# SamsungLabs/nb-asr

Hardware: AMD Instinct MI355X
Metric: utterances_per_sec (higher is better)
Workload: dtype f32

## Files before the change

### nb_asr_amd/csrc/gemm_pointwise.hip

```cpp
#include "storage.h"

namespace nbasr {

typedef float floatx4 __attribute__((ext_vector_type(4)));
typedef _Float16 pw_h2 __attribute__((ext_vector_type(2)));

constexpr int PW_M = 128, PW_N = 256, PW_K = 32;
constexpr int PW_THREADS = 512;

__device__ __forceinline__ float pw_load(const float* p) { return *p; }
__device__ __forceinline__ float pw_load(const bf16_t* p) { return __uint_as_float(static_cast<unsigned>(p->bits) << 16); }
__device__ __forceinline__ void pw_store(float* p, float v) { *p = v; }
__device__ __forceinline__ void pw_store(bf16_t* p, float v) { p->bits = static_cast<unsigned short>(pack_bf16x2(v, 0.f) & 0xffffu); }

template <int TERMS>
struct PwSteps {
    static constexpr int NS = TERMS;
    static constexpr int A_STEP = TERMS * 2 * 2 * PW_M * 16;
    static constexpr int X_STEP = TERMS * 2 * 2 * PW_N * 16;
    static constexpr int RING = 3;
    static constexpr int LDS = RING * (A_STEP + X_STEP);
    static constexpr int DMA_PER_WAVE = 3 * TERMS;
};

// ... 82 lines not shown


template <bool LNX, class T>
__device__ __forceinline__ void pw_fetch32(const T* __restrict__ x, int c_in, int frames, int ld, const LnRef& ln, float (&v)[PW_K])
{
    const int ci0 = blockIdx.y * PW_K, b = blockIdx.z;
    const int t = blockIdx.x * PW_N + threadIdx.x;
    const bool live = t < frames;
    const T* __restrict__ xb = x + static_cast<size_t>(b) * c_in * ld + t;
    float mean = 0.f, rstd = 0.f;
    if (LNX && live) {
        const float* st = ln.stats + static_cast<size_t>(b) * 2 * ld;
        mean = st[t]; rstd = st[ld + t];
    }
#pragma unroll
    for (int c = 0; c < PW_K; ++c) {
        const int ci = ci0 + c;
        v[c] = (live && ci < c_in) ? pw_load(xb + static_cast<size_t>(ci) * ld) : 0.f;
    }
    if (LNX) {
#pragma unroll
        for (int c = 0; c < PW_K; ++c) {
            const int ci = ci0 + c;
            if (live && ci < c_in) v[c] = ln_apply(v[c], mean, rstd, ln.gamma[ci], ln.beta[ci]);
        }
    }
}

template <bool LNX>
__global__ __launch_bounds__(256) void pw_tile_max_kernel(const float* __restrict__ x, float* __restrict__ partial, int c_in,
                                                          int frames, int ld, int n_ks, const LnRef ln)
{
    __shared__ float s_max[4];
    float v[PW_K];
    pw_fetch32<LNX>(x, c_in, frames, ld, ln, v);
    float m = 0.f;
#pragma unroll
    for (int c = 0; c < PW_K; ++c) m = fmaxf(m, fabsf(v[c]));
#pragma unroll
    for (int d = 32; d >= 1; d >>= 1) m = fmaxf(m, __shfl_xor(m, d));
    if ((threadIdx.x & 63) == 0) s_max[threadIdx.x >> 6] = m;
    __syncthreads();
    if (threadIdx.x == 0)
        partial[(static_cast<size_t>(blockIdx.z) * gridDim.x + blockIdx.x) * n_ks + blockIdx.y] = fmaxf(fmaxf(s_max[0], s_max[1]), fmaxf(s_max[2], s_max[3]));
}

template <class P, bool LNX>
__global__ __launch_bounds__(256) void pw_presplit_kernel(const typename P::act_t* __restrict__ x, unsigned char* __restrict__ image,
                                                          float* __restrict__ inv_scale, const float* __restrict__ partial,
                                                          int c_in, int frames, int ld, int n_ks, const LnRef ln)
{
    const int nt = blockIdx.x, ks = blockIdx.y, b = blockIdx.z;
    const int lane_t = threadIdx.x;
    float v[PW_K];
    pw_fetch32<LNX>(x, c_in, frames, ld, ln, v);
    float scale = 1.f;
    if constexpr (P::SCALED) {
        const float* __restrict__ pt = partial + (static_cast<size_t>(b) * gridDim.x + nt) * n_ks;
        float tile_max = 0.f;
        for (int i = threadIdx.x & 63; i < n_ks; i += 64) tile_max = fmaxf(tile_max, pt[i]);
#pragma unroll
        for (int d = 32; d >= 1; d >>= 1) tile_max = fmaxf(tile_max, __shfl_xor(tile_max, d));
        float inv;
        pw_pow2(tile_max, 14, scale, inv);
        if (threadIdx.x == 0 && ks == 0) inv_scale[static_cast<size_t>(b) * gridDim.x + nt] = inv;
    }
    unsigned char* step = image + ((static_cast<size_t>(b) * gridDim.x + nt) * n_ks + ks) * P::X_STEP;
#pragma unroll
    for (int bh = 0; bh < 4; ++bh) {
        u4v term[P::NS];
#pragma unroll
// ... 425 lines not shown
```

### nb_asr_amd/csrc/layernorm.hip

```cpp
#include "storage.h"

namespace nbasr {

constexpr int LN_ROWS = 16;
constexpr int LN_QS = 16;

template <typename T, bool MINMAX = false, int FR = Chunk<T>::FR>
__device__ __forceinline__ void tile_statistics(const T* x, int channels, int ld, float eps, size_t base, bool active,
                                                int row, int ql, float (*s_mean)[LN_QS * FR], float (*s_m2)[LN_QS * FR],
                                                float* s_cnt, float* s_mu, float* s_rstd,
                                                float (*s_lo)[LN_QS * FR] = nullptr, float (*s_hi)[LN_QS * FR] = nullptr)
{
    float shift[FR], s1[FR], s2[FR], lo[FR], hi[FR];
#pragma unroll
    for (int r = 0; r < FR; ++r) { shift[r] = 0.f; s1[r] = 0.f; s2[r] = 0.f; lo[r] = 3.0e38f; hi[r] = -3.0e38f; }
    int n = 0;
    if (active && row < channels) {
        load_frames<FR>(x + base + static_cast<size_t>(row) * ld, shift);
        auto fold = [&](const float (&e)[FR]) {
#pragma unroll
            for (int r = 0; r < FR; ++r) {
                const float d = e[r] - shift[r];
                s1[r] += d;
                s2[r] = __builtin_fmaf(d, d, s2[r]);
                if (MINMAX) { lo[r] = fminf(lo[r], e[r]); hi[r] = fmaxf(hi[r], e[r]); }
            }
            ++n;
        };
        int c = row;
        for (; c + 7 * LN_ROWS < channels; c += 8 * LN_ROWS) {
            float e[8][FR];
#pragma unroll
            for (int u = 0; u < 8; ++u) load_frames<FR>(x + base + static_cast<size_t>(c + u * LN_ROWS) * ld, e[u]);
#pragma unroll
            for (int u = 0; u < 8; ++u) fold(e[u]);
        }
        for (; c + 3 * LN_ROWS < channels; c += 4 * LN_ROWS) {
            float e[4][FR];
#pragma unroll
            for (int u = 0; u < 4; ++u) load_frames<FR>(x + base + static_cast<size_t>(c + u * LN_ROWS) * ld, e[u]);
#pragma unroll
            for (int u = 0; u < 4; ++u) fold(e[u]);
        }
        for (; c < channels; c += LN_ROWS) {
            float e[FR];
            load_frames<FR>(x + base + static_cast<size_t>(c) * ld, e);
            fold(e);
        }
    }
    const float fn = static_cast<float>(n);
#pragma unroll
    for (int r = 0; r < FR; ++r) {
        const float dm = n ? s1[r] / fn : 0.f;
        s_mean[row][ql * FR + r] = shift[r] + dm;
        s_m2[row][ql * FR + r] = n ? fmaxf(s2[r] - dm * s1[r], 0.f) : 0.f;
        if (MINMAX) { s_lo[row][ql * FR + r] = lo[r]; s_hi[row][ql * FR + r] = hi[r]; }
    }
    if (ql == 0) s_cnt[row] = fn;
    __syncthreads();

    if (threadIdx.x < LN_QS * FR) {
        const int col = threadIdx.x;
        float cnt = 0.f, mean = 0.f, m2 = 0.f;
#pragma unroll
        for (int k = 0; k < LN_ROWS; ++k) {
            const float nb = s_cnt[k];
            if (nb > 0.f) {
                const float tot = cnt + nb;
                const float delta = s_mean[k][col] - mean;
                mean += delta * (nb / tot);
                m2 += s_m2[k][col] + delta * delta * (cnt * nb / tot);
                cnt = tot;
            }
        }
        s_mu[col] = mean;
        s_rstd[col] = 1.0f / sqrtf(m2 / fmaxf(cnt, 1.f) + eps);
        if (MINMAX) {
            float l = s_lo[0][col], h = s_hi[0][col];
#pragma unroll
            for (int k = 1; k < LN_ROWS; ++k) { l = fminf(l, s_lo[k][col]); h = fmaxf(h, s_hi[k][col]); }
            s_lo[0][col] = l; s_hi[0][col] = h;
        }
    }
    __syncthreads();
}

template <typename TI, typename TO, bool ABSMAX>
__global__ __launch_bounds__(256) void layernorm_channels_kernel(
    const TI* x, const float* __restrict__ gamma, const float* __restrict__ beta,
    TO* y, int channels, int frames, int ld, float eps, unsigned* __restrict__ absmax)
{
    constexpr int FR = Chunk<TI>::FR;
    __shared__ float s_mean[LN_ROWS][LN_QS * FR];
    __shared__ float s_m2[LN_ROWS][LN_QS * FR];
// ... 88 lines not shown
    NBASR_REQUIRE(x && gamma && beta && y, NBASR_ENULL, "%s: NULL pointer", what);
    NBASR_REQUIRE(aligned16(x) && aligned16(y), NBASR_EALIGN, "%s: x, y must be 16-byte aligned", what);
    NBASR_REQUIRE(batch <= 65535, NBASR_EINVAL, "%s: batch %d > 65535", what, batch);
    NBASR_REQUIRE(!absmax || in_dtype == NBASR_F32, NBASR_EINVAL, "%s: the absmax by-product exists for fp32 tensors only", what);
    const int nq = ld / fr;
    const dim3 grid((nq + LN_QS - 1) / LN_QS, batch);
    if (in_dtype == NBASR_BF16) {
        if (out_dtype == NBASR_BF16)
            hipLaunchKernelGGL((layernorm_channels_kernel<bf16_t, bf16_t, false>), grid, dim3(256), 0, as_stream(stream),
                               static_cast<const bf16_t*>(x), gamma, beta, static_cast<bf16_t*>(y), channels, frames, ld, eps, static_cast<unsigned*>(nullptr));
        else
            hipLaunchKernelGGL((layernorm_channels_kernel<bf16_t, float, false>), grid, dim3(256), 0, as_stream(stream),
                               static_cast<const bf16_t*>(x), gamma, beta, static_cast<float*>(y), channels, frames, ld, eps, static_cast<unsigned*>(nullptr));
    } else if (absmax) {
        zero_async(absmax, sizeof(float) * batch, as_stream(stream));
        hipLaunchKernelGGL((layernorm_channels_kernel<float, float, true>), grid, dim3(256), 0, as_stream(stream),
                           static_cast<const float*>(x), gamma, beta, static_cast<float*>(y), channels, frames, ld, eps, reinterpret_cast<unsigned*>(absmax));
    } else {
        hipLaunchKernelGGL((layernorm_channels_kernel<float, float, false>), grid, dim3(256), 0, as_stream(stream),
                           static_cast<const float*>(x), gamma, beta, static_cast<float*>(y), channels, frames, ld, eps, static_cast<unsigned*>(nullptr));
    }
    return launch_status(what);
}

extern "C" int nbasr_layernorm_channels(const void* x, const float* gamma, const float* beta, void* y, float* absmax, int batch,
                                        int channels, int frames, int ld, float eps, int in_dtype, int out_dtype, nbasr_stream_t stream)
{
    clear_error();
    NBASR_REQUIRE(!absmax || (in_dtype == NBASR_F32 && out_dtype == NBASR_F32), NBASR_EINVAL,
                  "nbasr_layernorm_channels: the max|y| by-product exists for fp32 -> fp32 only");
    return layernorm_impl("nbasr_layernorm_channels", x, gamma, beta, y, absmax, batch, channels, frames, ld, eps, stream, in_dtype, out_dtype);
}

__global__ __launch_bounds__(256) void channel_stats_bound_kernel(const float* __restrict__ x, const float* __restrict__ gamma,
                                                                  const float* __restrict__ beta, float* __restrict__ stats,
                                                                  unsigned* __restrict__ bound, int channels, int frames, int ld, float eps)
{
    __shared__ float s_mean[LN_ROWS][LN_QS * 4];
    __shared__ float s_m2[LN_ROWS][LN_QS * 4];
    __shared__ float s_cnt[LN_ROWS];
    __shared__ float s_mu[LN_QS * 4];
    __shared__ float s_rstd[LN_QS * 4];
    __shared__ float s_gb[8];
    __shared__ float s_lo[LN_ROWS][LN_QS * 4];
    __shared__ float s_hi[LN_ROWS][LN_QS * 4];

    const int ql = threadIdx.x & (LN_QS - 1);
    const int row = threadIdx.x / LN_QS;
    const int nq = ld >> 2;
    const int q = blockIdx.x * LN_QS + ql;
    const int b = blockIdx.y;
    const bool active = q < nq;
    const size_t base = static_cast<size_t>(b) * channels * ld + static_cast<size_t>(q) * 4;

    float gm = 0.f, bm = 0.f;
    for (int c = threadIdx.x; c < channels; c += 256) { gm = fmaxf(gm, fabsf(gamma[c])); bm = fmaxf(bm, fabsf(beta[c])); }
#pragma unroll
    for (int d = 32; d >= 1; d >>= 1) { gm = fmaxf(gm, __shfl_xor(gm, d)); bm = fmaxf(bm, __shfl_xor(bm, d)); }
    if ((threadIdx.x & 63) == 0) { s_gb[threadIdx.x >> 6] = gm; s_gb[4 + (threadIdx.x >> 6)] = bm; }

    tile_statistics<float, true>(x, channels, ld, eps, base, active, row, ql, s_mean, s_m2, s_cnt, s_mu, s_rstd, s_lo, s_hi);
    gm = fmaxf(fmaxf(s_gb[0], s_gb[1]), fmaxf(s_gb[2], s_gb[3]));
    bm = fmaxf(fmaxf(s_gb[4], s_gb[5]), fmaxf(s_gb[6], s_gb[7]));

    float dev = 0.f;
    if (threadIdx.x < LN_QS * 4) {
        const int t = blockIdx.x * (LN_QS * 4) + threadIdx.x;
        if (t < ld) {
            const bool live = t < frames;
            float* srow = stats + static_cast<size_t>(b) * 2 * ld;
            srow[t] = live ? s_mu[threadIdx.x] : 0.f;
            srow[ld + t] = live ? s_rstd[threadIdx.x] : 0.f;
            if (live) dev = finite_abs(fmaxf(s_hi[0][threadIdx.x] - s_mu[threadIdx.x], s_mu[threadIdx.x] - s_lo[0][threadIdx.x]) * s_rstd[threadIdx.x]);
        }
    }
    if (threadIdx.x < 64) {
#pragma unroll
        for (int d = 32; d >= 1; d >>= 1) dev = fmaxf(dev, __shfl_xor(dev, d));
        if (threadIdx.x == 0) atomicMax(bound + b, __float_as_uint(finite_abs((dev * gm + bm) * 1.0001f)));
    }
}

template <bool NORM>
__global__ __launch_bounds__(256) void normalize_split_kernel(const float* __restrict__ x, const float* __restrict__ stats,
                                                              const float* __restrict__ gamma, const float* __restrict__ beta,
                                                              const float* __restrict__ bound, unsigned char* __restrict__ image,
                                                              int channels, int , int ld,
                                                              int bound_stride)
{
    typedef _Float16 halfx8 __attribute__((ext_vector_type(8)));
    constexpr int SPLIT_PITCH = 68;
    __shared__ __attribute__((aligned(16))) unsigned char s_tile[4][2][4 * SPLIT_PITCH * 16];
    const int ql = threadIdx.x & 63, wv = threadIdx.x >> 6, oct0 = wv + 4 * blockIdx.z;
    const int nq = ld >> 2;
    const int q = blockIdx.x * 64 + ql;
    const int b = blockIdx.y;
    const int n_groups = (channels + 15) >> 4;
    const size_t rows = static_cast<size_t>(ld) + 1;
    unsigned char* const img_b = image + static_cast<size_t>(b) * n_groups * 4 * rows * 16;
    if (blockIdx.x == 0 && blockIdx.z == 0) {
        const uint4 z = make_uint4(0u, 0u, 0u, 0u);
        for (int pl = threadIdx.x; pl < n_groups * 4; pl += 256) *reinterpret_cast<uint4*>(img_b + static_cast<size_t>(pl) * rows * 16) = z;
    }
    if (blockIdx.x * 64 >= nq) return;
    const bool inside = q < nq;
    float scale = 1.f;
    {
        const unsigned bits = __float_as_uint(bound[static_cast<size_t>(b) * bound_stride]);
        const int e = static_cast<int>((bits >> 23) & 0xffu);
        int k = (bits & 0x7fffffffu) ? (127 + 14) - e : 0;
        k = k > 126 ? 126 : (k < -126 ? -126 : k);
        scale = __uint_as_float(static_cast<unsigned>(127 + k) << 23);
// ... 67 lines not shown
            const int f = 64 * k + ql;
            if (blockIdx.x * 256 + f < ld) {
                *reinterpret_cast<halfx8*>(plane_hi + f * 16) = hi;
                *reinterpret_cast<halfx8*>(plane_lo + f * 16) = lo;
            }
        }
        asm volatile("s_waitcnt lgkmcnt(0)" ::: "memory");
#pragma unroll
        for (int c = 0; c < 8; ++c) cur[c] = nxt[c];
    }
}

static int split_grid_z(int tiles, int batch)
{
    const long long wgs = static_cast<long long>(tiles) * batch;
    int z = 4;
    while (z < 16 && wgs * z < 512) z *= 2;
    return z;
}

extern "C" int nbasr_layernorm_split_image(const float* x, const float* gamma, const float* beta, float* stats, float* bound,
                                           void* image, int batch, int channels, int frames, int ld, float eps,
                                           nbasr_stream_t stream)
{
    clear_error();
    NBASR_REQUIRE(batch >= 0 && channels > 0 && frames >= 0, NBASR_EINVAL, "nbasr_layernorm_split_image: bad sizes");
    NBASR_REQUIRE(ld >= frames && ld % 4 == 0, NBASR_EALIGN, "nbasr_layernorm_split_image: ld=%d must be >= frames=%d and a multiple of 4", ld, frames);
    if (batch == 0 || ld == 0) return NBASR_OK;
    NBASR_REQUIRE(x && gamma && beta && stats && bound && image, NBASR_ENULL, "nbasr_layernorm_split_image: NULL pointer");
    NBASR_REQUIRE(aligned16(x) && aligned16(stats) && aligned16(image), NBASR_EALIGN, "nbasr_layernorm_split_image: x, stats, image must be 16-byte aligned");
    NBASR_REQUIRE(batch <= 65535, NBASR_EINVAL, "nbasr_layernorm_split_image: batch %d > 65535", batch);
    zero_async(bound, sizeof(float) * batch, as_stream(stream));
    const int nq = ld / 4;
    hipLaunchKernelGGL(channel_stats_bound_kernel, dim3((nq + LN_QS - 1) / LN_QS, batch), dim3(256), 0, as_stream(stream),
                       x, gamma, beta, stats, reinterpret_cast<unsigned*>(bound), channels, frames, ld, eps);
    hipLaunchKernelGGL(normalize_split_kernel<true>, dim3((nq + 63) / 64, batch, split_grid_z((nq + 63) / 64, batch)), dim3(256), 0, as_stream(stream),
                       x, stats, gamma, beta, bound, static_cast<unsigned char*>(image), channels, frames, ld, 1);
    return launch_status("nbasr_layernorm_split_image");
}

__global__ __launch_bounds__(256) void input_range_kernel(const float* __restrict__ x, unsigned* __restrict__ range,
                                                          int channels, int frames, int ld)
{
    __shared__ float s_max[4][256];
    __shared__ unsigned s_bad[4];
    const int b = blockIdx.y;
    const int lane = threadIdx.x & 63, slice = threadIdx.x >> 6;
    const int t0 = (blockIdx.x * 64 + lane) * 4;
    float m[4] = {0.f, 0.f, 0.f, 0.f};
    unsigned bad = 0u;
    if (t0 < frames) {
        const float* col = x + static_cast<size_t>(b) * channels * ld + t0;
        const bool whole = t0 + 4 <= ld && ld % 4 == 0 && (reinterpret_cast<size_t>(x) & 15) == 0;
        for (int c = slice; c < channels; c += 4) {
            float v[4] = {0.f, 0.f, 0.f, 0.f};
            if (whole) {
                const float4 q = *reinterpret_cast<const float4*>(col + static_cast<size_t>(c) * ld);
                v[0] = q.x; v[1] = q.y; v[2] = q.z; v[3] = q.w;
            } else {
#pragma unroll
                for (int r = 0; r < 4; ++r) if (t0 + r < frames) v[r] = col[static_cast<size_t>(c) * ld + r];
            }
#pragma unroll
            for (int r = 0; r < 4; ++r) {
                const float a = fabsf(v[r]);
                if (t0 + r < frames) {
                    if (!(a <= 3.4028234664e38f)) bad = 1u;
                    else m[r] = fmaxf(m[r], a);
                }
            }
        }
    }
#pragma unroll
    for (int r = 0; r < 4; ++r) s_max[slice][lane * 4 + r] = m[r];
#pragma unroll
    for (int d = 32; d >= 1; d >>= 1) bad |= __shfl_xor(bad, d);
    if (lane == 0) s_bad[slice] = bad;
    __syncthreads();
    const int t = blockIdx.x * 256 + threadIdx.x;
    const float fmax_ = fmaxf(fmaxf(s_max[0][threadIdx.x], s_max[1][threadIdx.x]), fmaxf(s_max[2][threadIdx.x], s_max[3][threadIdx.x]));
    float hi = fmax_, lo = (t < frames && fmax_ > 0.f) ? fmax_ : __uint_as_float(0x7f800000u);
#pragma unroll
    for (int d = 32; d >= 1; d >>= 1) {
        hi = fmaxf(hi, __shfl_xor(hi, d));
        lo = fminf(lo, __shfl_xor(lo, d));
    }
    if (lane == 0) {
        atomicMax(range + 4 * b, __float_as_uint(hi));
        atomicMin(range + 4 * b + 1, __float_as_uint(lo));
        if (slice == 0 && (s_bad[0] | s_bad[1] | s_bad[2] | s_bad[3])) atomicOr(range + 4 * b + 2, 0x3f800000u);
    }
}

__global__ void input_range_init_kernel(unsigned* __restrict__ range, int batch)
{
    const int b = blockIdx.x * blockDim.x + threadIdx.x;
    if (b < batch) { range[4 * b] = 0u; range[4 * b + 1] = 0x7f800000u; range[4 * b + 2] = 0u; range[4 * b + 3] = 0u; }
}

extern "C" int nbasr_input_range(const float* x, float* range, int batch, int channels, int frames, int ld, nbasr_stream_t stream)
{
    clear_error();
    NBASR_REQUIRE(batch >= 0 && channels > 0 && frames >= 0 && ld >= frames, NBASR_EINVAL, "nbasr_input_range: bad sizes");
    if (batch == 0) return NBASR_OK;
    NBASR_REQUIRE(range, NBASR_ENULL, "nbasr_input_range: range is NULL");
    NBASR_REQUIRE(batch <= 65535, NBASR_EINVAL, "nbasr_input_range: batch %d > 65535", batch);
    hipLaunchKernelGGL(input_range_init_kernel, dim3((batch + 255) / 256), dim3(256), 0, as_stream(stream), reinterpret_cast<unsigned*>(range), batch);
    if (frames > 0) {
        NBASR_REQUIRE(x, NBASR_ENULL, "nbasr_input_range: x is NULL");
        hipLaunchKernelGGL(input_range_kernel, dim3((frames + 255) / 256, batch), dim3(256), 0, as_stream(stream), x,
                           reinterpret_cast<unsigned*>(range), channels, frames, ld);
    }
    return launch_status("nbasr_input_range");
}

extern "C" int nbasr_split_image_ranged(const float* x, const float* x_range, void* image, int batch, int channels, int frames,
                                        int ld, nbasr_stream_t stream)
{
    clear_error();
    NBASR_REQUIRE(batch >= 0 && channels > 0 && frames >= 0, NBASR_EINVAL, "nbasr_split_image_ranged: bad sizes");
    NBASR_REQUIRE(ld >= frames && ld % 4 == 0, NBASR_EALIGN, "nbasr_split_image_ranged: ld=%d must be >= frames=%d and a multiple of 4", ld, frames);
    if (batch == 0 || ld == 0) return NBASR_OK;
    NBASR_REQUIRE(x && x_range && image, NBASR_ENULL, "nbasr_split_image_ranged: NULL pointer");
    NBASR_REQUIRE(aligned16(x) && aligned16(image), NBASR_EALIGN, "nbasr_split_image_ranged: x, image must be 16-byte aligned");
    NBASR_REQUIRE(batch <= 65535, NBASR_EINVAL, "nbasr_split_image_ranged: batch %d > 65535", batch);
    const int nq = ld / 4;
    hipLaunchKernelGGL(normalize_split_kernel<false>, dim3((nq + 63) / 64, batch, split_grid_z((nq + 63) / 64, batch)), dim3(256), 0, as_stream(stream),
                       x, static_cast<const float*>(nullptr), static_cast<const float*>(nullptr), static_cast<const float*>(nullptr),
                       x_range, static_cast<unsigned char*>(image), channels, frames, ld, 4);
    return launch_status("nbasr_split_image_ranged");
}

extern "C" int nbasr_channel_stats(const void* x, float* stats, int batch, int channels, int frames, int ld, float eps, int dtype,
                                     nbasr_stream_t stream)
{
    clear_error();
    NBASR_REQUIRE(dtype == NBASR_F32 || dtype == NBASR_BF16, NBASR_EINVAL, "nbasr_channel_stats: unknown dtype %d", dtype);
    NBASR_REQUIRE(batch >= 0 && channels > 0 && frames >= 0, NBASR_EINVAL, "nbasr_channel_stats: bad sizes");
    const int fr = dtype == NBASR_BF16 ? 8 : 4;
    NBASR_REQUIRE(ld >= frames && ld % fr == 0, NBASR_EALIGN, "nbasr_channel_stats: ld=%d must be >= frames=%d and a multiple of %d", ld, frames, fr);
    if (batch == 0 || ld == 0) return NBASR_OK;
    NBASR_REQUIRE(x && stats, NBASR_ENULL, "nbasr_channel_stats: NULL pointer");
    NBASR_REQUIRE(aligned16(x) && aligned16(stats), NBASR_EALIGN, "nbasr_channel_stats: x, stats must be 16-byte aligned");
// ... 129 lines not shown
```

### nb_asr_amd/csrc/lstm.hip

```cpp
#include "common.h"

#include <cstdlib>
#include <mutex>
#include <vector>

namespace nbasr {

constexpr int NBASR_MAX_DEVICES = 64;

typedef float floatx4 __attribute__((ext_vector_type(4)));

int lstm_input_projection(const float* x, const float* w_ih, const float* b_ih, const float* b_hh, float* gates,
                          int batch, int c_in, int frames, int ld, int rows4h, LnRef ln, hipStream_t stream);

__device__ __forceinline__ float sigmoidf_(float v) { return 1.0f / (1.0f + expf(-v)); }

constexpr int LSTM_WAVES = 8;
constexpr int LSTM_CHUNKS = 4;

constexpr int LSTMP_HU = 8;

__global__ __launch_bounds__(256) void lstm_pack_whh_kernel(const float* __restrict__ w_hh, float4* __restrict__ packed, int hidden,
                                                            int slices, int kchunks_p)
{
// ... 54 lines not shown
            for (int c = 0; c < LSTM_CHUNKS; ++c) {
#pragma unroll
                for (int m = 0; m < 2; ++m) acc[m] = __builtin_amdgcn_mfma_f32_16x16x4f32(wv[c][m].x, hv[c].x, acc[m], 0, 0, 0);
#pragma unroll
                for (int m = 0; m < 2; ++m) acc[m] = __builtin_amdgcn_mfma_f32_16x16x4f32(wv[c][m].y, hv[c].y, acc[m], 0, 0, 0);
#pragma unroll
                for (int m = 0; m < 2; ++m) acc[m] = __builtin_amdgcn_mfma_f32_16x16x4f32(wv[c][m].z, hv[c].z, acc[m], 0, 0, 0);
#pragma unroll
                for (int m = 0; m < 2; ++m) acc[m] = __builtin_amdgcn_mfma_f32_16x16x4f32(wv[c][m].w, hv[c].w, acc[m], 0, 0, 0);
            }
        }
    }
#pragma unroll
    for (int m = 0; m < 2; ++m)
#pragma unroll
        for (int r = 0; r < 4; ++r) red[wave][m][r][lane] = acc[m][r];
    __syncthreads();

    if (!e_ok) return;
    const int mt = jj >> 2, pl = (jj & 3) * 16 + bb;
#pragma unroll
    for (int g = 0; g < 4; ++g) {
        float s = red[0][mt][g][pl];
#pragma unroll
        for (int w = 1; w < LSTM_WAVES; ++w) s += red[w][mt][g][pl];
        pre[g] += s;
    }
    const float c_new = sigmoidf_(pre[1]) * c_prev + sigmoidf_(pre[0]) * tanhf(pre[2]);
    const float h_new = sigmoidf_(pre[3]) * tanhf(c_new);
    cell[static_cast<size_t>(eb) * hidden + ej] = c_new;
    h_out[(static_cast<size_t>(eb) * frames + t) * hidden + ej] = h_new;
}

template <bool BCT>
__global__ __launch_bounds__(256) void head_kernel(
    const float* __restrict__ h, const float* __restrict__ w, const float* __restrict__ bias,
    float* __restrict__ out, int rows, int features, int classes, int frames, int ld, const LnRef ln)
{
    const int lane = threadIdx.x & 63, wave = threadIdx.x >> 6;
    const int i16 = lane & 15, kq = lane >> 4;
    const int r0 = (blockIdx.x * 4 + wave) * 16;
    if (r0 >= rows) return;

    floatx4 acc[4], part[4];
#pragma unroll
    for (int n = 0; n < 4; ++n) { acc[n] = floatx4{0.f, 0.f, 0.f, 0.f}; part[n] = floatx4{0.f, 0.f, 0.f, 0.f}; }

    const int row = r0 + i16;
    const bool row_ok = row < rows;
    const int kchunks = (features + 15) / 16;
    for (int c = 0; c < kchunks; ++c) {
        if ((c & 7) == 0 && c) {
#pragma unroll
            for (int n = 0; n < 4; ++n) { acc[n] += part[n]; part[n] = floatx4{0.f, 0.f, 0.f, 0.f}; }
        }
        const int k = c * 16 + kq * 4;
        const bool kok = k < features;
        float av[4] = {0.f, 0.f, 0.f, 0.f};
        if (row_ok && kok) {
            if (!BCT) {
                const float4 v = *reinterpret_cast<const float4*>(h + static_cast<size_t>(row) * features + k);
                av[0] = v.x; av[1] = v.y; av[2] = v.z; av[3] = v.w;
            } else {
                const int bb = row / frames, tt = row - bb * frames;
                const float* p = h + (static_cast<size_t>(bb) * features + k) * ld + tt;
#pragma unroll
                for (int e = 0; e < 4; ++e) av[e] = p[static_cast<size_t>(e) * ld];
                if (ln.stats) {
                    const float* st = ln.stats + static_cast<size_t>(bb) * 2 * ld;
                    const float mean = st[tt], rstd = st[ld + tt];
#pragma unroll
                    for (int e = 0; e < 4; ++e) av[e] = ln_apply(av[e], mean, rstd, ln.gamma[k + e], ln.beta[k + e]);
                }
            }
        }
#pragma unroll
        for (int n = 0; n < 4; ++n) {
            const int cls = n * 16 + i16;
            float4 wv = make_float4(0.f, 0.f, 0.f, 0.f);
            if (cls < classes && kok) wv = *reinterpret_cast<const float4*>(w + static_cast<size_t>(cls) * features + k);
            part[n] = __builtin_amdgcn_mfma_f32_16x16x4f32(av[0], wv.x, part[n], 0, 0, 0);
            part[n] = __builtin_amdgcn_mfma_f32_16x16x4f32(av[1], wv.y, part[n], 0, 0, 0);
            part[n] = __builtin_amdgcn_mfma_f32_16x16x4f32(av[2], wv.z, part[n], 0, 0, 0);
            part[n] = __builtin_amdgcn_mfma_f32_16x16x4f32(av[3], wv.w, part[n], 0, 0, 0);
        }
    }
#pragma unroll
    for (int n = 0; n < 4; ++n) acc[n] += part[n];
#pragma unroll
    for (int n = 0; n < 4; ++n) {
        const int cls = n * 16 + i16;
        if (cls >= classes) continue;
        const float bv = bias[cls];
#pragma unroll
        for (int r = 0; r < 4; ++r) {
            const int rr = r0 + kq * 4 + r;
            if (rr < rows) out[static_cast<size_t>(rr) * classes + cls] = acc[n][r] + bv;
        }
    }
}

constexpr int LSTMS_QUADS = LSTM_WAVES * LSTM_CHUNKS * 4;
constexpr int LSTMS_IMAGE_FLOATS = LSTMS_QUADS * 16 * 4;
constexpr int LSTMS_HEADER_WORDS = 64;
constexpr unsigned long long LSTMS_TIMEOUT_TICKS = 100000000ull;

typedef unsigned lstm_u4 __attribute__((ext_vector_type(4)));

__device__ __forceinline__ unsigned lstm_tag(int t) { return (static_cast<unsigned>((t >> 1) + 1) & 1u) << 30; }

__global__ __launch_bounds__(64 * LSTM_WAVES) void lstm_seq_kernel(
    const float* __restrict__ gates_in,
    const float4* __restrict__ wp,
    float* __restrict__ cell, float* __restrict__ h_out, unsigned* status, float* hx,
    int batch, int frames, int hidden, int kchunks_p, int flags)
{
    __shared__ float4 red[2][LSTM_WAVES][2][64];
    __shared__ int stop;
    if ((flags & NBASR_LSTM_SEQ_INJECT_FAULT) && blockIdx.x == 0) return;

    const int lane = threadIdx.x & 63, wave = __builtin_amdgcn_readfirstlane(threadIdx.x >> 6);
    const int i16 = lane & 15, kq = lane >> 4;
    const int slice = blockIdx.x, tile = blockIdx.y;
    const int b0 = tile * 16;
    if (threadIdx.x == 0) stop = 0;

    float4 wv[LSTM_CHUNKS][2];
    {
        const bool mine = wave * LSTM_CHUNKS < kchunks_p;
        const float4* wslice = wp + (static_cast<size_t>(slice) * kchunks_p + (mine ? wave * LSTM_CHUNKS : 0)) * 2 * 64 + lane;
#pragma unroll
// ... 269 lines not shown
    } else {
        hipLaunchKernelGGL(lstm_seq_kernel, grid, block, 0, as_stream(stream), gates_ws, static_cast<const float4*>(packed_whh), cell_ws, h_out,
                           words, hx, batch, frames, hidden, lstm_kchunks_p(hidden), flags);
    }
    e = hipEventRecord(done, as_stream(stream));
    if (e != hipSuccess) { set_error("nbasr_lstm_recurrence_seq: hipEventRecord: %s", hipGetErrorString(e)); return static_cast<int>(e); }
    return launch_status("nbasr_lstm_recurrence_seq");
}

extern "C" int nbasr_lstm_seq_status(const void* seq_ws, nbasr_stream_t stream)
{
    clear_error();
    NBASR_REQUIRE(seq_ws, NBASR_ENULL, "nbasr_lstm_seq_status: NULL pointer");
    unsigned word = 0;
    hipError_t e = hipMemcpyAsync(&word, seq_ws, sizeof(word), hipMemcpyDeviceToHost, as_stream(stream));
    if (e == hipSuccess) e = hipStreamSynchronize(as_stream(stream));
    if (e != hipSuccess) { set_error("nbasr_lstm_seq_status: %s", hipGetErrorString(e)); return static_cast<int>(e); }
    NBASR_REQUIRE(word == 0, NBASR_EINVAL, "nbasr_lstm_seq_status: a step of the one-launch recurrence timed out waiting for its peers "
                  "(status %u): the grid was not co-resident", word);
    return NBASR_OK;
}

extern "C" int nbasr_linear_head(const float* h, const float* w, const float* bias, float* logits, int rows,
                                 int features, int classes, nbasr_stream_t stream)
{
    clear_error();
    NBASR_REQUIRE(rows >= 0 && features > 0 && classes > 0 && classes <= 64, NBASR_EINVAL,
                  "nbasr_linear_head: rows=%d features=%d classes=%d (classes must be <= 64)", rows, features, classes);
    if (rows == 0) return NBASR_OK;
    NBASR_REQUIRE(h && w && bias && logits, NBASR_ENULL, "nbasr_linear_head: NULL pointer");
    NBASR_REQUIRE(features % 4 == 0 && aligned16(h) && aligned16(w), NBASR_EALIGN,
                  "nbasr_linear_head: features must be a multiple of 4 and h, w 16-byte aligned");
    if (rows == 0) return NBASR_OK;
    hipLaunchKernelGGL(head_kernel<false>, dim3((rows + 63) / 64), dim3(256), 0, as_stream(stream),
                       h, w, bias, logits, rows, features, classes, 0, 0, LnRef{nullptr, nullptr, nullptr});
    return launch_status("nbasr_linear_head");
}

extern "C" int nbasr_linear_head_bct(const float* x, const float* w, const float* bias, float* logits, int batch,
                                     int features, int frames, int ld, int classes, const nbasr_deferred_ln* ln,
                                     nbasr_stream_t stream)
{
    clear_error();
    NBASR_REQUIRE(batch >= 0 && features > 0 && frames >= 0 && ld >= frames && classes > 0 && classes <= 64, NBASR_EINVAL,
                  "nbasr_linear_head_bct: bad sizes (classes must be <= 64)");
    if (batch == 0 || frames == 0) return NBASR_OK;
    NBASR_REQUIRE(x && w && bias && logits, NBASR_ENULL, "nbasr_linear_head_bct: NULL pointer");
    NBASR_REQUIRE(features % 4 == 0 && aligned16(w), NBASR_EALIGN, "nbasr_linear_head_bct: features must be a multiple of 4, w 16-byte aligned");
    NBASR_REQUIRE(!ln || (ln->stats && ln->gamma && ln->beta), NBASR_ENULL, "nbasr_linear_head_bct: deferred LayerNorm needs stats, gamma and beta");
    const long long rows = static_cast<long long>(batch) * frames;
    if (rows == 0) return NBASR_OK;
    hipLaunchKernelGGL(head_kernel<true>, dim3(static_cast<unsigned>((rows + 63) / 64)), dim3(256), 0, as_stream(stream),
                       x, w, bias, logits, static_cast<int>(rows), features, classes, frames, ld, ln_ref(ln, true));
    return launch_status("nbasr_linear_head_bct");
}
```

Measured before the change: 11470.

## Vectorize tile-max fetch, widen stats/range kernels with XCD tiling, LDS-stage head GEMM

The pointwise tile-max kernel gains a float4 fast path for aligned inputs. The channel-stats and input-range kernels move to wider 512/256-thread blocks with XCD-contiguous tile remapping, and the range kernel gets a deeper load unroll. The linear head kernel is rewritten to stage weight and activation tiles in LDS, with register prefetch of the next K block, so weights are reused across waves. Together these aim to cut memory traffic and latency in several small kernels, at the cost of more LDS, extra synchronisation and more code complexity.

```diff
diff --git a/nb_asr_amd/csrc/gemm_pointwise.hip b/nb_asr_amd/csrc/gemm_pointwise.hip
--- a/nb_asr_amd/csrc/gemm_pointwise.hip
+++ b/nb_asr_amd/csrc/gemm_pointwise.hip
@@ -138,11 +138,45 @@
                                                           int frames, int ld, int n_ks, const LnRef ln)
 {
     __shared__ float s_max[4];
-    float v[PW_K];
-    pw_fetch32<LNX>(x, c_in, frames, ld, ln, v);
     float m = 0.f;
-#pragma unroll
-    for (int c = 0; c < PW_K; ++c) m = fmaxf(m, fabsf(v[c]));
+    if (ld % 4 == 0 && ((reinterpret_cast<size_t>(x) | (LNX ? reinterpret_cast<size_t>(ln.stats) : 0)) & 15) == 0) {
+        const int ci0 = blockIdx.y * PW_K + (threadIdx.x >> 6) * (PW_K / 4), b = blockIdx.z;
+        const int t0 = blockIdx.x * PW_N + (threadIdx.x & 63) * 4;
+        if (t0 < frames) {
+            const float* __restrict__ xb = x + static_cast<size_t>(b) * c_in * ld + t0;
+            float4 q[PW_K / 4];
+#pragma unroll
+            for (int c = 0; c < PW_K / 4; ++c) {
+                const int ci = ci0 + c;
+                q[c] = ci < c_in ? *reinterpret_cast<const float4*>(xb + static_cast<size_t>(ci) * ld) : make_float4(0.f, 0.f, 0.f, 0.f);
+            }
+            float mean[4] = {0.f, 0.f, 0.f, 0.f}, rstd[4] = {0.f, 0.f, 0.f, 0.f};
+            if (LNX) {
+                const float* st = ln.stats + static_cast<size_t>(b) * 2 * ld + t0;
+                const float4 mu = *reinterpret_cast<const float4*>(st), rs = *reinterpret_cast<const float4*>(st + ld);
+                mean[0] = mu.x; mean[1] = mu.y; mean[2] = mu.z; mean[3] = mu.w;
+                rstd[0] = rs.x; rstd[1] = rs.y; rstd[2] = rs.z; rstd[3] = rs.w;
+            }
+#pragma unroll
+            for (int c = 0; c < PW_K / 4; ++c) {
+                const int ci = ci0 + c;
+                const float e[4] = {q[c].x, q[c].y, q[c].z, q[c].w};
+                float g = 0.f, be = 0.f;
+                if (LNX && ci < c_in) { g = ln.gamma[ci]; be = ln.beta[ci]; }
+#pragma unroll
+                for (int r = 0; r < 4; ++r) {
+                    float v = e[r];
+                    if (LNX) v = ln_apply(v, mean[r], rstd[r], g, be);
+                    if (t0 + r < frames && ci < c_in) m = fmaxf(m, fabsf(v));
+                }
+            }
+        }
+    } else {
+        float v[PW_K];
+        pw_fetch32<LNX>(x, c_in, frames, ld, ln, v);
+#pragma unroll
+        for (int c = 0; c < PW_K; ++c) m = fmaxf(m, fabsf(v[c]));
+    }
 #pragma unroll
     for (int d = 32; d >= 1; d >>= 1) m = fmaxf(m, __shfl_xor(m, d));
     if ((threadIdx.x & 63) == 0) s_max[threadIdx.x >> 6] = m;
diff --git a/nb_asr_amd/csrc/layernorm.hip b/nb_asr_amd/csrc/layernorm.hip
--- a/nb_asr_amd/csrc/layernorm.hip
+++ b/nb_asr_amd/csrc/layernorm.hip
@@ -5,11 +5,11 @@
 constexpr int LN_ROWS = 16;
 constexpr int LN_QS = 16;
 
-template <typename T, bool MINMAX = false, int FR = Chunk<T>::FR>
+template <typename T, bool MINMAX = false, int QS = LN_QS, int FR = Chunk<T>::FR>
 __device__ __forceinline__ void tile_statistics(const T* x, int channels, int ld, float eps, size_t base, bool active,
-                                                int row, int ql, float (*s_mean)[LN_QS * FR], float (*s_m2)[LN_QS * FR],
+                                                int row, int ql, float (*s_mean)[QS * FR], float (*s_m2)[QS * FR],
                                                 float* s_cnt, float* s_mu, float* s_rstd,
-                                                float (*s_lo)[LN_QS * FR] = nullptr, float (*s_hi)[LN_QS * FR] = nullptr)
+                                                float (*s_lo)[QS * FR] = nullptr, float (*s_hi)[QS * FR] = nullptr)
 {
     float shift[FR], s1[FR], s2[FR], lo[FR], hi[FR];
 #pragma unroll
@@ -59,7 +59,7 @@
     if (ql == 0) s_cnt[row] = fn;
     __syncthreads();
 
-    if (threadIdx.x < LN_QS * FR) {
+    if (threadIdx.x < QS * FR) {
         const int col = threadIdx.x;
         float cnt = 0.f, mean = 0.f, m2 = 0.f;
 #pragma unroll
@@ -214,40 +214,49 @@
     return layernorm_impl("nbasr_layernorm_channels", x, gamma, beta, y, absmax, batch, channels, frames, ld, eps, stream, in_dtype, out_dtype);
 }
 
-__global__ __launch_bounds__(256) void channel_stats_bound_kernel(const float* __restrict__ x, const float* __restrict__ gamma,
-                                                                  const float* __restrict__ beta, float* __restrict__ stats,
-                                                                  unsigned* __restrict__ bound, int channels, int frames, int ld, float eps)
-{
-    __shared__ float s_mean[LN_ROWS][LN_QS * 4];
-    __shared__ float s_m2[LN_ROWS][LN_QS * 4];
+__device__ __forceinline__ int xcd_contiguous_tile(int id, int n)
+{
+    const int xq = n >> 3, xr = n & 7, xcd = id & 7;
+    return (xcd < xr ? xcd * (xq + 1) : xr * (xq + 1) + (xcd - xr) * xq) + (id >> 3);
+}
+
+constexpr int SB_QS = 32;
+constexpr int SB_THREADS = LN_ROWS * SB_QS;
+__global__ __launch_bounds__(SB_THREADS) void channel_stats_bound_kernel(const float* __restrict__ x, const float* __restrict__ gamma,
+                                                                         const float* __restrict__ beta, float* __restrict__ stats,
+                                                                         unsigned* __restrict__ bound, int channels, int frames, int ld, float eps)
+{
+    constexpr int COLS = SB_QS * 4;
+    __shared__ float s_mean[LN_ROWS][COLS];
+    __shared__ float s_m2[LN_ROWS][COLS];
     __shared__ float s_cnt[LN_ROWS];
-    __shared__ float s_mu[LN_QS * 4];
-    __shared__ float s_rstd[LN_QS * 4];
-    __shared__ float s_gb[8];
-    __shared__ float s_lo[LN_ROWS][LN_QS * 4];
-    __shared__ float s_hi[LN_ROWS][LN_QS * 4];
-
-    const int ql = threadIdx.x & (LN_QS - 1);
-    const int row = threadIdx.x / LN_QS;
+    __shared__ float s_mu[COLS];
+    __shared__ float s_rstd[COLS];
+    __shared__ float s_gb[2 * (SB_THREADS / 64)];
+    __shared__ float s_dev[COLS / 64];
+    __shared__ float s_lo[LN_ROWS][COLS];
+    __shared__ float s_hi[LN_ROWS][COLS];
+
+    const int ql = threadIdx.x & (SB_QS - 1);
+    const int row = threadIdx.x / SB_QS;
     const int nq = ld >> 2;
-    const int q = blockIdx.x * LN_QS + ql;
-    const int b = blockIdx.y;
+    const int tile_id = xcd_contiguous_tile(blockIdx.x + gridDim.x * blockIdx.y, gridDim.x * gridDim.y);
+    const int b = tile_id / static_cast<int>(gridDim.x), tile = tile_id - b * static_cast<int>(gridDim.x);
+    const int q = tile * SB_QS + ql;
     const bool active = q < nq;
     const size_t base = static_cast<size_t>(b) * channels * ld + static_cast<size_t>(q) * 4;
 
     float gm = 0.f, bm = 0.f;
-    for (int c = threadIdx.x; c < channels; c += 256) { gm = fmaxf(gm, fabsf(gamma[c])); bm = fmaxf(bm, fabsf(beta[c])); }
+    for (int c = threadIdx.x; c < channels; c += SB_THREADS) { gm = fmaxf(gm, fabsf(gamma[c])); bm = fmaxf(bm, fabsf(beta[c])); }
 #pragma unroll
     for (int d = 32; d >= 1; d >>= 1) { gm = fmaxf(gm, __shfl_xor(gm, d)); bm = fmaxf(bm, __shfl_xor(bm, d)); }
-    if ((threadIdx.x & 63) == 0) { s_gb[threadIdx.x >> 6] = gm; s_gb[4 + (threadIdx.x >> 6)] = bm; }
-
-    tile_statistics<float, true>(x, channels, ld, eps, base, active, row, ql, s_mean, s_m2, s_cnt, s_mu, s_rstd, s_lo, s_hi);
-    gm = fmaxf(fmaxf(s_gb[0], s_gb[1]), fmaxf(s_gb[2], s_gb[3]));
-    bm = fmaxf(fmaxf(s_gb[4], s_gb[5]), fmaxf(s_gb[6], s_gb[7]));
+    if ((threadIdx.x & 63) == 0) { s_gb[threadIdx.x >> 6] = gm; s_gb[SB_THREADS / 64 + (threadIdx.x >> 6)] = bm; }
+
+    tile_statistics<float, true, SB_QS>(x, channels, ld, eps, base, active, row, ql, s_mean, s_m2, s_cnt, s_mu, s_rstd, s_lo, s_hi);
 
     float dev = 0.f;
-    if (threadIdx.x < LN_QS * 4) {
-        const int t = blockIdx.x * (LN_QS * 4) + threadIdx.x;
+    if (threadIdx.x < COLS) {
+        const int t = tile * COLS + threadIdx.x;
         if (t < ld) {
             const bool live = t < frames;
             float* srow = stats + static_cast<size_t>(b) * 2 * ld;
@@ -255,11 +264,19 @@
             srow[ld + t] = live ? s_rstd[threadIdx.x] : 0.f;
             if (live) dev = finite_abs(fmaxf(s_hi[0][threadIdx.x] - s_mu[threadIdx.x], s_mu[threadIdx.x] - s_lo[0][threadIdx.x]) * s_rstd[threadIdx.x]);
         }
-    }
-    if (threadIdx.x < 64) {
 #pragma unroll
         for (int d = 32; d >= 1; d >>= 1) dev = fmaxf(dev, __shfl_xor(dev, d));
-        if (threadIdx.x == 0) atomicMax(bound + b, __float_as_uint(finite_abs((dev * gm + bm) * 1.0001f)));
+        if ((threadIdx.x & 63) == 0) s_dev[threadIdx.x >> 6] = dev;
+    }
+    __syncthreads();
+    if (threadIdx.x == 0) {
+#pragma unroll
+        for (int i = 1; i < SB_THREADS / 64; ++i) { gm = fmaxf(gm, s_gb[i]); bm = fmaxf(bm, s_gb[SB_THREADS / 64 + i]); }
+        float bnd = 0.f;
+#pragma unroll
+        for (int i = 0; i < COLS / 64; ++i)
+            if (tile * COLS + i * 64 < ld) bnd = fmaxf(bnd, finite_abs((s_dev[i] * gm + bm) * 1.0001f));
+        atomicMax(bound + b, __float_as_uint(bnd));
     }
 }
 
@@ -393,63 +410,83 @@
     NBASR_REQUIRE(batch <= 65535, NBASR_EINVAL, "nbasr_layernorm_split_image: batch %d > 65535", batch);
     zero_async(bound, sizeof(float) * batch, as_stream(stream));
     const int nq = ld / 4;
-    hipLaunchKernelGGL(channel_stats_bound_kernel, dim3((nq + LN_QS - 1) / LN_QS, batch), dim3(256), 0, as_stream(stream),
+    hipLaunchKernelGGL(channel_stats_bound_kernel, dim3((nq + SB_QS - 1) / SB_QS, batch), dim3(SB_THREADS), 0, as_stream(stream),
                        x, gamma, beta, stats, reinterpret_cast<unsigned*>(bound), channels, frames, ld, eps);
     hipLaunchKernelGGL(normalize_split_kernel<true>, dim3((nq + 63) / 64, batch, split_grid_z((nq + 63) / 64, batch)), dim3(256), 0, as_stream(stream),
                        x, stats, gamma, beta, bound, static_cast<unsigned char*>(image), channels, frames, ld, 1);
     return launch_status("nbasr_layernorm_split_image");
 }
 
-__global__ __launch_bounds__(256) void input_range_kernel(const float* __restrict__ x, unsigned* __restrict__ range,
-                                                          int channels, int frames, int ld)
-{
-    __shared__ float s_max[4][256];
-    __shared__ unsigned s_bad[4];
-    const int b = blockIdx.y;
-    const int lane = threadIdx.x & 63, slice = threadIdx.x >> 6;
-    const int t0 = (blockIdx.x * 64 + lane) * 4;
+constexpr int IR_QS = 32, IR_SLICES = 8, IR_DEPTH = 10;
+__global__ __launch_bounds__(IR_QS * IR_SLICES) void input_range_kernel(const float* __restrict__ x, unsigned* __restrict__ range,
+                                                                       int channels, int frames, int ld)
+{
+    constexpr int COLS = IR_QS * 4;
+    __shared__ float s_max[IR_SLICES][COLS];
+    __shared__ unsigned s_bad[IR_QS * IR_SLICES / 64];
+    const int tile_id = xcd_contiguous_tile(blockIdx.x + gridDim.x * blockIdx.y, gridDim.x * gridDim.y);
+    const int b = tile_id / static_cast<int>(gridDim.x), tile = tile_id - b * static_cast<int>(gridDim.x);
+    const int ql = threadIdx.x & (IR_QS - 1), slice = threadIdx.x / IR_QS;
+    const int t0 = (tile * IR_QS + ql) * 4;
     float m[4] = {0.f, 0.f, 0.f, 0.f};
     unsigned bad = 0u;
     if (t0 < frames) {
         const float* col = x + static_cast<size_t>(b) * channels * ld + t0;
         const bool whole = t0 + 4 <= ld && ld % 4 == 0 && (reinterpret_cast<size_t>(x) & 15) == 0;
-        for (int c = slice; c < channels; c += 4) {
-            float v[4] = {0.f, 0.f, 0.f, 0.f};
-            if (whole) {
-                const float4 q = *reinterpret_cast<const float4*>(col + static_cast<size_t>(c) * ld);
-                v[0] = q.x; v[1] = q.y; v[2] = q.z; v[3] = q.w;
-            } else {
-#pragma unroll
-                for (int r = 0; r < 4; ++r) if (t0 + r < frames) v[r] = col[static_cast<size_t>(c) * ld + r];
-            }
-#pragma unroll
-            for (int r = 0; r < 4; ++r) {
-                const float a = fabsf(v[r]);
-                if (t0 + r < frames) {
-                    if (!(a <= 3.4028234664e38f)) bad = 1u;
-                    else m[r] = fmaxf(m[r], a);
+        for (int c0 = slice; c0 < channels; c0 += IR_SLICES * IR_DEPTH) {
+            float v[IR_DEPTH][4];
+#pragma unroll
+            for (int u = 0; u < IR_DEPTH; ++u) {
+                const int c = c0 + u * IR_SLICES;
+#pragma unroll
+                for (int r = 0; r < 4; ++r) v[u][r] = 0.f;
+                if (c < channels) {
+                    if (whole) {
+                        const float4 q = *reinterpret_cast<const float4*>(col + static_cast<size_t>(c) * ld);
+                        v[u][0] = q.x; v[u][1] = q.y; v[u][2] = q.z; v[u][3] = q.w;
+                    } else {
+#pragma unroll
+                        for (int r = 0; r < 4; ++r) if (t0 + r < frames) v[u][r] = col[static_cast<size_t>(c) * ld + r];
+                    }
                 }
             }
-        }
-    }
-#pragma unroll
-    for (int r = 0; r < 4; ++r) s_max[slice][lane * 4 + r] = m[r];
+#pragma unroll
+            for (int u = 0; u < IR_DEPTH; ++u) {
+#pragma unroll
+                for (int r = 0; r < 4; ++r) {
+                    const float a = fabsf(v[u][r]);
+                    if (t0 + r < frames) {
+                        if (!(a <= 3.4028234664e38f)) bad = 1u;
+                        else m[r] = fmaxf(m[r], a);
+                    }
+                }
+            }
+        }
+    }
+#pragma unroll
+    for (int r = 0; r < 4; ++r) s_max[slice][ql * 4 + r] = m[r];
 #pragma unroll
     for (int d = 32; d >= 1; d >>= 1) bad |= __shfl_xor(bad, d);
-    if (lane == 0) s_bad[slice] = bad;
+    if ((threadIdx.x & 63) == 0) s_bad[threadIdx.x >> 6] = bad;
     __syncthreads();
-    const int t = blockIdx.x * 256 + threadIdx.x;
-    const float fmax_ = fmaxf(fmaxf(s_max[0][threadIdx.x], s_max[1][threadIdx.x]), fmaxf(s_max[2][threadIdx.x], s_max[3][threadIdx.x]));
+    if (threadIdx.x >= COLS) return;
+    const int t = tile * COLS + threadIdx.x;
+    float fmax_ = s_max[0][threadIdx.x];
+#pragma unroll
+    for (int k = 1; k < IR_SLICES; ++k) fmax_ = fmaxf(fmax_, s_max[k][threadIdx.x]);
     float hi = fmax_, lo = (t < frames && fmax_ > 0.f) ? fmax_ : __uint_as_float(0x7f800000u);
 #pragma unroll
     for (int d = 32; d >= 1; d >>= 1) {
         hi = fmaxf(hi, __shfl_xor(hi, d));
         lo = fminf(lo, __shfl_xor(lo, d));
     }
-    if (lane == 0) {
+    if ((threadIdx.x & 63) == 0) {
         atomicMax(range + 4 * b, __float_as_uint(hi));
         atomicMin(range + 4 * b + 1, __float_as_uint(lo));
-        if (slice == 0 && (s_bad[0] | s_bad[1] | s_bad[2] | s_bad[3])) atomicOr(range + 4 * b + 2, 0x3f800000u);
+        bad = 0u;
+#pragma unroll
+        for (int k = 0; k < IR_QS * IR_SLICES / 64; ++k) bad |= s_bad[k];
+        if (threadIdx.x == 0 && bad) atomicOr(range + 4 * b + 2, 0x3f800000u);
     }
 }
 
@@ -469,7 +506,7 @@
     hipLaunchKernelGGL(input_range_init_kernel, dim3((batch + 255) / 256), dim3(256), 0, as_stream(stream), reinterpret_cast<unsigned*>(range), batch);
     if (frames > 0) {
         NBASR_REQUIRE(x, NBASR_ENULL, "nbasr_input_range: x is NULL");
-        hipLaunchKernelGGL(input_range_kernel, dim3((frames + 255) / 256, batch), dim3(256), 0, as_stream(stream), x,
+        hipLaunchKernelGGL(input_range_kernel, dim3((frames + IR_QS * 4 - 1) / (IR_QS * 4), batch), dim3(IR_QS * IR_SLICES), 0, as_stream(stream), x,
                            reinterpret_cast<unsigned*>(range), channels, frames, ld);
     }
     return launch_status("nbasr_input_range");
diff --git a/nb_asr_amd/csrc/lstm.hip b/nb_asr_amd/csrc/lstm.hip
--- a/nb_asr_amd/csrc/lstm.hip
+++ b/nb_asr_amd/csrc/lstm.hip
@@ -110,71 +110,110 @@
     h_out[(static_cast<size_t>(eb) * frames + t) * hidden + ej] = h_new;
 }
 
+constexpr int HEAD_ROWS = 32;
+constexpr int HEAD_KB = 128;
+constexpr int HEAD_PITCH = HEAD_KB + 4;
+constexpr int HEAD_THREADS = 512;
 template <bool BCT>
-__global__ __launch_bounds__(256) void head_kernel(
+__global__ __launch_bounds__(HEAD_THREADS) void head_kernel(
     const float* __restrict__ h, const float* __restrict__ w, const float* __restrict__ bias,
     float* __restrict__ out, int rows, int features, int classes, int frames, int ld, const LnRef ln)
 {
+    __shared__ __attribute__((aligned(16))) float s_h[HEAD_ROWS][HEAD_PITCH];
+    __shared__ __attribute__((aligned(16))) float s_w[64][HEAD_PITCH];
     const int lane = threadIdx.x & 63, wave = threadIdx.x >> 6;
+    const int rt = wave >> 2, n = wave & 3;
     const int i16 = lane & 15, kq = lane >> 4;
-    const int r0 = (blockIdx.x * 4 + wave) * 16;
-    if (r0 >= rows) return;
-
-    floatx4 acc[4], part[4];
-#pragma unroll
-    for (int n = 0; n < 4; ++n) { acc[n] = floatx4{0.f, 0.f, 0.f, 0.f}; part[n] = floatx4{0.f, 0.f, 0.f, 0.f}; }
-
-    const int row = r0 + i16;
-    const bool row_ok = row < rows;
+    const int r0 = blockIdx.x * HEAD_ROWS;
+    const bool tile_live = r0 + rt * 16 < rows && n * 16 < classes;
+
+    const int sq = threadIdx.x & 31, sr = threadIdx.x >> 5;
+    const int br = threadIdx.x & 31, bk = threadIdx.x >> 5;
+    const float* hrow = h;
+    bool brow_ok = false;
+    float mean = 0.f, rstd = 0.f;
+    if (BCT && r0 + br < rows) {
+        const int row = r0 + br, bb = row / frames, tt = row - bb * frames;
+        brow_ok = true;
+        hrow = h + static_cast<size_t>(bb) * features * ld + tt;
+        if (ln.stats) {
+            const float* st = ln.stats + static_cast<size_t>(bb) * 2 * ld;
+            mean = st[tt]; rstd = st[ld + tt];
+        }
+    }
+    float4 fw[4], fh[2];
+    float fb[8];
+    auto fetch = [&](int k0) {
+        const int k = k0 + sq * 4;
+#pragma unroll
+        for (int j = 0; j < 4; ++j) {
+            const int cls = sr + 16 * j;
+            fw[j] = (cls < classes && k < features) ? *reinterpret_cast<const float4*>(w + static_cast<size_t>(cls) * features + k)
+                                                    : make_float4(0.f, 0.f, 0.f, 0.f);
+        }
+        if (!BCT) {
+#pragma unroll
+            for (int j = 0; j < 2; ++j) {
+                const int row = r0 + sr + 16 * j;
+                fh[j] = (row < rows && k < features) ? *reinterpret_cast<const float4*>(h + static_cast<size_t>(row) * features + k)
+                                                     : make_float4(0.f, 0.f, 0.f, 0.f);
+            }
+        } else {
+#pragma unroll
+            for (int j = 0; j < 8; ++j) {
+                const int kk = k0 + bk + 16 * j;
+                fb[j] = 0.f;
+                if (brow_ok && kk < features) {
+                    fb[j] = hrow[static_cast<size_t>(kk) * ld];
+                    if (ln.stats) fb[j] = ln_apply(fb[j], mean, rstd, ln.gamma[kk], ln.beta[kk]);
+                }
+            }
+        }
+    };
+    auto stage = [&]() {
+#pragma unroll
+        for (int j = 0; j < 4; ++j) *reinterpret_cast<float4*>(&s_w[sr + 16 * j][sq * 4]) = fw[j];
+        if (!BCT) {
+#pragma unroll
+            for (int j = 0; j < 2; ++j) *reinterpret_cast<float4*>(&s_h[sr + 16 * j][sq * 4]) = fh[j];
+        } else {
+#pragma unroll
+            for (int j = 0; j < 8; ++j) s_h[br][bk + 16 * j] = fb[j];
+        }
+    };
+
+    floatx4 acc = floatx4{0.f, 0.f, 0.f, 0.f}, part = floatx4{0.f, 0.f, 0.f, 0.f};
     const int kchunks = (features + 15) / 16;
-    for (int c = 0; c < kchunks; ++c) {
-        if ((c & 7) == 0 && c) {
-#pragma unroll
-            for (int n = 0; n < 4; ++n) { acc[n] += part[n]; part[n] = floatx4{0.f, 0.f, 0.f, 0.f}; }
-        }
-        const int k = c * 16 + kq * 4;
-        const bool kok = k < features;
-        float av[4] = {0.f, 0.f, 0.f, 0.f};
-        if (row_ok && kok) {
-            if (!BCT) {
-                const float4 v = *reinterpret_cast<const float4*>(h + static_cast<size_t>(row) * features + k);
-                av[0] = v.x; av[1] = v.y; av[2] = v.z; av[3] = v.w;
-            } else {
-                const int bb = row / frames, tt = row - bb * frames;
-                const float* p = h + (static_cast<size_t>(bb) * features + k) * ld + tt;
-#pragma unroll
-                for (int e = 0; e < 4; ++e) av[e] = p[static_cast<size_t>(e) * ld];
-                if (ln.stats) {
-                    const float* st = ln.stats + static_cast<size_t>(bb) * 2 * ld;
-                    const float mean = st[tt], rstd = st[ld + tt];
-#pragma unroll
-                    for (int e = 0; e < 4; ++e) av[e] = ln_apply(av[e], mean, rstd, ln.gamma[k + e], ln.beta[k + e]);
-                }
-            }
-        }
-#pragma unroll
-        for (int n = 0; n < 4; ++n) {
-            const int cls = n * 16 + i16;
-            float4 wv = make_float4(0.f, 0.f, 0.f, 0.f);
-            if (cls < classes && kok) wv = *reinterpret_cast<const float4*>(w + static_cast<size_t>(cls) * features + k);
-            part[n] = __builtin_amdgcn_mfma_f32_16x16x4f32(av[0], wv.x, part[n], 0, 0, 0);
-            part[n] = __builtin_amdgcn_mfma_f32_16x16x4f32(av[1], wv.y, part[n], 0, 0, 0);
-            part[n] = __builtin_amdgcn_mfma_f32_16x16x4f32(av[2], wv.z, part[n], 0, 0, 0);
-            part[n] = __builtin_amdgcn_mfma_f32_16x16x4f32(av[3], wv.w, part[n], 0, 0, 0);
-        }
-    }
-#pragma unroll
-    for (int n = 0; n < 4; ++n) acc[n] += part[n];
-#pragma unroll
-    for (int n = 0; n < 4; ++n) {
-        const int cls = n * 16 + i16;
-        if (cls >= classes) continue;
-        const float bv = bias[cls];
-#pragma unroll
-        for (int r = 0; r < 4; ++r) {
-            const int rr = r0 + kq * 4 + r;
-            if (rr < rows) out[static_cast<size_t>(rr) * classes + cls] = acc[n][r] + bv;
-        }
+    const float* const ha = &s_h[rt * 16 + i16][kq * 4];
+    const float* const wb = &s_w[n * 16 + i16][kq * 4];
+    fetch(0);
+    for (int k0 = 0; k0 < features; k0 += HEAD_KB) {
+        if (k0) __syncthreads();
+        stage();
+        __syncthreads();
+        if (k0 + HEAD_KB < features) fetch(k0 + HEAD_KB);
+        if (!tile_live) continue;
+        if (k0) { acc += part; part = floatx4{0.f, 0.f, 0.f, 0.f}; }
+#pragma unroll
+        for (int u = 0; u < HEAD_KB / 16; ++u) {
+            if (k0 / 16 + u < kchunks) {
+                const floatx4 av = *reinterpret_cast<const floatx4*>(ha + u * 16);
+                const floatx4 wv = *reinterpret_cast<const floatx4*>(wb + u * 16);
+                part = __builtin_amdgcn_mfma_f32_16x16x4f32(av[0], wv[0], part, 0, 0, 0);
+                part = __builtin_amdgcn_mfma_f32_16x16x4f32(av[1], wv[1], part, 0, 0, 0);
+                part = __builtin_amdgcn_mfma_f32_16x16x4f32(av[2], wv[2], part, 0, 0, 0);
+                part = __builtin_amdgcn_mfma_f32_16x16x4f32(av[3], wv[3], part, 0, 0, 0);
+            }
+        }
+    }
+    acc += part;
+    const int cls = n * 16 + i16;
+    if (!tile_live || cls >= classes) return;
+    const float bv = bias[cls];
+#pragma unroll
+    for (int r = 0; r < 4; ++r) {
+        const int rr = r0 + rt * 16 + kq * 4 + r;
+        if (rr < rows) out[static_cast<size_t>(rr) * classes + cls] = acc[r] + bv;
     }
 }
 
@@ -510,7 +549,7 @@
     NBASR_REQUIRE(features % 4 == 0 && aligned16(h) && aligned16(w), NBASR_EALIGN,
                   "nbasr_linear_head: features must be a multiple of 4 and h, w 16-byte aligned");
     if (rows == 0) return NBASR_OK;
-    hipLaunchKernelGGL(head_kernel<false>, dim3((rows + 63) / 64), dim3(256), 0, as_stream(stream),
+    hipLaunchKernelGGL(head_kernel<false>, dim3((rows + HEAD_ROWS - 1) / HEAD_ROWS), dim3(HEAD_THREADS), 0, as_stream(stream),
                        h, w, bias, logits, rows, features, classes, 0, 0, LnRef{nullptr, nullptr, nullptr});
     return launch_status("nbasr_linear_head");
 }
@@ -528,7 +567,7 @@
     NBASR_REQUIRE(!ln || (ln->stats && ln->gamma && ln->beta), NBASR_ENULL, "nbasr_linear_head_bct: deferred LayerNorm needs stats, gamma and beta");
     const long long rows = static_cast<long long>(batch) * frames;
     if (rows == 0) return NBASR_OK;
-    hipLaunchKernelGGL(head_kernel<true>, dim3(static_cast<unsigned>((rows + 63) / 64)), dim3(256), 0, as_stream(stream),
+    hipLaunchKernelGGL(head_kernel<true>, dim3(static_cast<unsigned>((rows + HEAD_ROWS - 1) / HEAD_ROWS)), dim3(HEAD_THREADS), 0, as_stream(stream),
                        x, w, bias, logits, static_cast<int>(rows), features, classes, frames, ld, ln_ref(ln, true));
     return launch_status("nbasr_linear_head_bct");
 }
```

After: 11500 (median of 6 runs). Within noise of the previous version (+0.3%).
